# marja-w/gan-des-midi-music-gen

Measured on AMD Instinct MI355X. Metric: GAN training samples/sec (G+D step), higher is better.
Workload: dtype bf16; 1 GPU; SIMNN G/D iteration, synthetic 128x256 spectrogram windows; per_gpu_batch=256, global_batch=256, mode=faithful, parallelism=dp1

## Files before the change

### gan_des_midi_music_gen_amd/_lib.py

```python
import ctypes
import os
import threading

_PKG = os.path.dirname(os.path.abspath(__file__))
_TAG = os.environ.get("GDM_LIB_TAG", "")
LIB_PATH = os.path.join(_PKG, "libgdm_hip" + (f"_{_TAG}" if _TAG else "") + ".so")

F32, BF16 = 0, 1
ACT_NONE, ACT_RELU, ACT_LEAKY, ACT_SIGMOID = 0, 1, 2, 3
CRITERIA = {"bce": 0, "mse": 1, "l1": 2}
PCM_U8, PCM_S16, PCM_S24, PCM_S32, PCM_F32 = range(5)
PCM_BYTES = (1, 2, 3, 4, 4)

_c = ctypes
_P, _I, _L, _F, _Z = _c.c_void_p, _c.c_int, _c.c_int64, _c.c_float, _c.c_size_t

class LinearBnJob(_c.Structure):
    _fields_ = [(n, _P) for n in ("x", "w", "bias", "gamma", "beta", "running_mean", "running_var",
                                  "num_batches_tracked", "y_out", "out", "save_mean", "save_invstd")] + \
               [(n, _I) for n in ("M", "N", "K", "groups", "stat_repeats")]


class DcnnAdam(_c.Structure):
    _fields_ = [("param", _P * 6), ("exp_avg", _P * 6), ("exp_avg_sq", _P * 6), ("hyper", _P), ("done", _P)]


class ConcatJob(_c.Structure):
    _fields_ = [("a", _P), ("b", _P), ("out", _P), ("M", _I), ("Ka", _I), ("Kb", _I)]


SIGNATURES = {
    "gdm_last_error": (_c.c_char_p, []),
    "gdm_version": (_I, []),
    "gdm_arch": (_c.c_char_p, []),
    "gdm_build_flavor": (_I, []),
    "gdm_gemm": (_I, [_P, _I, _L, _L, _P, _I, _L, _L, _P, _I, _L, _L, _I, _I, _I, _P, _P, _I, _F, _I, _I, _P, _Z, _P]),
    "gdm_gemm_plan": (_I, [_P, _I, _L, _L, _P, _I, _L, _L, _P, _I, _L, _L, _I, _I, _I, _P, _I, _I, _P]),
    "gdm_bce_with_logits": (_I, [_P, _F, _I, _F, _P, _P, _I, _I, _P]),
    "gdm_criterion_loss": (_I, [_P, _F, _I, _I, _F, _P, _P, _I, _P]),
    "gdm_adam_step": (_I, [_P, _P, _P, _P, _L, _I, _F, _F, _F, _F, _F, _P]),
    "gdm_adam_step_dev": (_I, [_P, _P, _P, _P, _L, _P, _P]),
    "gdm_adam_step_dev_pc": (_I, [_P, _P, _P, _P, _I, _I, _I, _P, _I, _P, _I, _P]),
    "gdm_stft_frames": (_I, [_P, _I, _L, _L, _I, _I, _I, _P, _P]),
    "gdm_power_spectrum": (_I, [_P, _L, _I, _I, _P, _P]),
    "gdm_power_to_db": (_I, [_P, _I, _I, _I, _F, _F, _P, _P]),
    "gdm_pcm_to_float": (_I, [_P, _I, _I, _I, _L, _L, _L, _P, _P]),
    "gdm_pcm_stft_frames": (_I, [_P, _I, _I, _I, _L, _L, _L, _I, _L, _L, _I, _I, _I, _P, _P]),
    "gdm_bn_workspace_bytes": (_Z, [_I, _I]),
    "gdm_bn_act_fwd": (_I, [_P, _I, _I, _P, _P, _P, _P, _P, _F, _F, _I, _P, _I, _P, _P, _I, _P, _Z, _P]),
    "gdm_bn_act_bwd": (_I, [_P, _P, _I, _P, _I, _I, _P, _P, _P, _I, _P, _P, _P, _P, _Z, _P]),
    "gdm_bn_stats": (_I, [_P, _I, _I, _P, _P, _P, _F, _F, _P, _P, _P, _Z, _P]),
    "gdm_bn_partial_chunks": (_I, [_I]),
# ... 104 lines not shown
```

### gan_des_midi_music_gen_amd/csrc/gemm.hip

```cpp
#include "gemm_common.h"

namespace {

constexpr int BM = 64, BN = 64, NT = 256;

template <typename CT> struct GemmCfg;
template <> struct GemmCfg<float> { static constexpr int KT = 32, LD = 34; };
template <> struct GemmCfg<__bf16> { static constexpr int KT = 64, LD = 72; };

template <typename CT, typename TA, typename TB>
__global__ __launch_bounds__(NT) void gemm_kernel(GemmArgs g) {
  constexpr int KT = GemmCfg<CT>::KT, LD = GemmCfg<CT>::LD;
  __shared__ __attribute__((aligned(16))) CT smem[(BM + BN) * LD];
  CT* As = smem;
  CT* Bs = smem + BM * LD;
  const int t = threadIdx.x, l = t & 63, w = t >> 6, wm = w >> 1, wn = w & 1;
  const int lr = l & 15, lg = l >> 4;
  const int m0 = blockIdx.y * BM, n0 = blockIdx.x * BN;
  const int kbeg = blockIdx.z * g.k_per_split;
  const int kend = min(g.K, kbeg + g.k_per_split);
  const TA* __restrict__ A = (const TA*)g.A;
  const TB* __restrict__ B = (const TB*)g.B;
  const bool a_kfast = (g.sak == 1), b_kfast = (g.sbk == 1);
  f32x4 acc[2][2];
// ... 210 lines not shown
      gdm_set_error("gdm_gemm: split_k=%d needs %zu workspace bytes, got %zu", p.split_k, p.ws_bytes, workspace_bytes);
      return GDM_EWORKSPACE;
    }
  }
  GemmArgs g{A, sam, sak, B, sbk, sbn, C, c_dtype, scm, scn, M, N, K, bias_n, bias_m, act, slope,
             p.split_k, p.k_per_split, (float*)workspace};
  hipStream_t s = (hipStream_t)stream;
  if (p.kernel == GDM_GEMM_KERNEL_FAST_K32 || p.kernel == GDM_GEMM_KERNEL_FAST_K64) {
    rc = gdm_gemm_bf16_fast_launch(g, a_dtype, b_dtype, p, s);
    if (rc != GDM_OK) return rc;
    return launch_splitk_reduce(g, p, s);
  }
  return p.kernel == GDM_GEMM_KERNEL_BF16 ? launch_gemm<__bf16>(g, p, a_dtype, b_dtype, s)
                                          : launch_gemm<float>(g, p, a_dtype, b_dtype, s);
}
```

### gan_des_midi_music_gen_amd/csrc/gemm_bf16.hip

```cpp
#include "gemm_common.h"

namespace {

constexpr int BM = 128, BN = 128;

inline bool operand_ok(const void* p, int dtype, int64_t s_row, int64_t s_k, int rows, int K, bool* kmaj) {
  const int64_t esz = dtype == GDM_BF16 ? 2 : 4, epc = 16 / esz;
  if (((uintptr_t)p & 15) != 0) return false;
  if (s_k == 1 && s_row >= 1 && (s_row * esz) % 16 == 0 && K % epc == 0) {
    *kmaj = true;
    return ((int64_t)(rows - 1) * s_row + K) * esz < ((int64_t)1 << 31);
  }
  if (s_row == 1 && s_k >= 1 && (s_k * esz) % 16 == 0 && rows % epc == 0) {
    *kmaj = false;
    return ((int64_t)(K - 1) * s_k + rows) * esz < ((int64_t)1 << 31);
  }
  return false;
}

}

bool gdm_gemm_bf16_fast_ok(const GemmArgs& g, int a_dtype, int b_dtype, bool* a_kmaj, bool* b_kmaj) {
  if (!operand_ok(g.A, a_dtype, g.sam, g.sak, g.M, g.K, a_kmaj)) return false;
  if (!operand_ok(g.B, b_dtype, g.sbn, g.sbk, g.N, g.K, b_kmaj)) return false;
// ... 4 lines not shown
    if (g.bias_n && ((uintptr_t)g.bias_n & 15) != 0) return false;
  }
  if ((int64_t)g.M * g.N < 64 * 64) return false;
  return true;
}

bool gdm_gemm_bf16_fast_deep(int M, int N, int split_k, int k_per_split) {
  const int MT = (M + BM - 1) / BM, NTl = (N + BN - 1) / BN;
  const int outer = NTl * split_k;
  bool deep = split_k > 1 && (int64_t)outer * MT <= 512 && k_per_split >= 256;
  static const int force = GDM_TUNABLE("GDM_GEMM_VARIANT", -1);
  if (force >= 0) deep = force == 1;
  return deep;
}

int gdm_gemm_bf16_fast_launch(const GemmArgs& g, int a_dtype, int b_dtype, const GemmPlan& p, hipStream_t s) {
  const int MT = (g.M + BM - 1) / BM, NTl = (g.N + BN - 1) / BN;
  const int outer = NTl * g.split_k;
  dim3 grid((unsigned)(((outer + 7) / 8) * 8 * MT));
  const bool deep = p.kernel == GDM_GEMM_KERNEL_FAST_K64;
  auto* launch = a_dtype == GDM_BF16 ? (deep ? gdm_gemm_bf16_kt64_bf16a : gdm_gemm_bf16_kt32_bf16a)
                                     : (deep ? gdm_gemm_bf16_kt64_f32a : gdm_gemm_bf16_kt32_f32a);
  launch(g, p.a_kmaj, b_dtype, p.b_kmaj, grid, s);
  GDM_LAUNCH_OK("gdm_gemm(bf16 fast path)");
  return GDM_OK;
}
```

### gan_des_midi_music_gen_amd/csrc/gemm_bf16_kernel.h

```cpp
#pragma once
#include <type_traits>
#include "buffer_ops.h"
#include "gemm_common.h"

namespace {

constexpr int BM = 128, BN = 128, NT = 256;

__device__ __forceinline__ void wave_lds_sync() {
  __builtin_amdgcn_fence(__ATOMIC_RELEASE, "wavefront");
  __builtin_amdgcn_wave_barrier();
  __builtin_amdgcn_fence(__ATOMIC_ACQUIRE, "wavefront");
}

template <int ACT> __device__ __forceinline__ float act_const(float v, float slope) {
  if constexpr (ACT == GDM_ACT_RELU) return v > 0.f ? v : 0.f;
  else if constexpr (ACT == GDM_ACT_LEAKY) return v > 0.f ? v : v * slope;
  else if constexpr (ACT == GDM_ACT_SIGMOID) return 1.0f / (1.0f + expf(-v));
  else return v;
}

template <int KT> __device__ __forceinline__ int kswz(int row) { return KT == 64 ? ((row >> 1) & 7) : ((row >> 1) & 2); }
__device__ __forceinline__ int rswz(int k) { return (k & 3) | ((k >> 1) & 4); }

// ... 19 lines not shown
    if constexpr (KMAJ) {
      constexpr int CPR = KT / EPC;
      rl = c / CPR; kl = (c % CPR) * EPC;
      ln.off[i] = (uint32_t)(((int64_t)(r0 + rl) * ld + kl) * (int64_t)sizeof(T));
      ln.lds[i] = rl * KT + 8 * ((kl >> 3) ^ kswz<KT>(rl)) + (kl & 7);
    } else {
      constexpr int CPK = 128 / EPC;
      kl = c / CPK; rl = (c % CPK) * EPC;
      ln.off[i] = (uint32_t)(((int64_t)kl * ld + r0 + rl) * (int64_t)sizeof(T));
      ln.lds[i] = kl * 128 + (rl ^ (16 * rswz(kl)));
    }
    ln.kl[i] = (r0 + rl < rows) ? kl : -1;
  }
}

template <typename T, int KT, bool KMAJ>
__device__ __forceinline__ void stage_load(Stage<T, KT>& st, const Lane<T, KT>& ln, rsrc_t rs, int64_t ld, int k0,
                                           int kend) {
  const uint32_t kbytes = (uint32_t)((KMAJ ? (int64_t)k0 : (int64_t)k0 * ld) * (int64_t)sizeof(T));
#pragma unroll
  for (int i = 0; i < Stage<T, KT>::N; ++i) {
    const bool ok = ln.kl[i] >= 0 && k0 + ln.kl[i] < kend;
    st.v[i] = __builtin_bit_cast(f32x4, __builtin_amdgcn_raw_buffer_load_b128(rs, ok ? kbytes + ln.off[i] : BUF_OOB, 0, 0));
  }
}

template <typename T, int KT>
__device__ __forceinline__ void stage_store(const Stage<T, KT>& st, const Lane<T, KT>& ln, __bf16* __restrict__ img) {
#pragma unroll
  for (int i = 0; i < Stage<T, KT>::N; ++i) {
    if constexpr (sizeof(T) == 2) {
      *(f32x4*)(img + ln.lds[i]) = st.v[i];
    } else {
      bf16x4 h;
#pragma unroll
      for (int e = 0; e < 4; ++e) h[e] = (__bf16)st.v[i][e];
      *(bf16x4*)(img + ln.lds[i]) = h;
    }
// ... 3 lines not shown
template <int KT, bool KMAJ>
__device__ __forceinline__ bf16x8 frag_read(const __bf16* __restrict__ img, int row0, int kk, int lr, int lg) {
  if constexpr (KMAJ) {
    const int row = row0 + lr;
    return *(const bf16x8*)&img[row * KT + 8 * ((4 * kk + lg) ^ kswz<KT>(row))];
  } else {
    const int q = lr >> 2, p = lr & 3;
    const int kr = 32 * kk + 8 * lg + q;
    const int n = (row0 + 4 * p) ^ (16 * (q | (4 * (lg & 1))));
    const bf16x4 lo = lds_tr16(&img[kr * 128 + n]);
    const bf16x4 hi = lds_tr16(&img[(kr + 4) * 128 + n]);
    return __builtin_shufflevector(lo, hi, 0, 1, 2, 3, 4, 5, 6, 7);
  }
}

template <typename TA, bool A_KMAJ, typename TB, bool B_KMAJ, int KT, int DEPTH>
__global__ __launch_bounds__(NT) void gemm_bf16_fast(GemmArgs g) {
  constexpr int IMG = 128 * KT;
  __shared__ __attribute__((aligned(16))) __bf16 smem[2 * DEPTH * IMG];
  const int t = threadIdx.x, l = t & 63, w = t >> 6, wm = w >> 1, wn = w & 1;
  const int lr = l & 15, lg = l >> 4;
  const int MT = (g.M + BM - 1) / BM, NTl = (g.N + BN - 1) / BN;
  const int id = blockIdx.x;
  const int grp = id / (8 * MT), within = id % (8 * MT);
  const int outer = grp * 8 + (within & 7), mt = within >> 3;
  if (outer >= NTl * g.split_k) return;
  const int nt = outer % NTl, zs = outer / NTl;
  const int m0 = mt * BM, n0 = nt * BN;
  const int kstep = KT * g.split_k;
  const int kbeg = zs * KT;
  const int kend = g.K;
  const int64_t lda = A_KMAJ ? g.sam : g.sak;
  const int64_t ldb = B_KMAJ ? g.sbn : g.sbk;
  const rsrc_t ra = make_rsrc(g.A, (uint32_t)((A_KMAJ ? (int64_t)(g.M - 1) * lda + g.K : (int64_t)(g.K - 1) * lda + g.M) *
// ... 13 lines not shown

  auto multiply = [&](const __bf16* As, const __bf16* Bs) {
#pragma unroll
    for (int kk = 0; kk < KT / 32; ++kk) {
      bf16x8 a[4], b[4];
#pragma unroll
      for (int i = 0; i < 4; ++i) a[i] = frag_read<KT, A_KMAJ>(As, wm * 64 + 16 * i, kk, lr, lg);
#pragma unroll
      for (int j = 0; j < 4; ++j) b[j] = frag_read<KT, B_KMAJ>(Bs, wn * 64 + 16 * j, kk, lr, lg);
#pragma unroll
      for (int i = 0; i < 4; ++i)
#pragma unroll
        for (int j = 0; j < 4; ++j) acc[i][j] = mfma16(b[j], a[i], acc[i][j]);
    }
  };
  Stage<TA, KT> sa[DEPTH];
  Stage<TB, KT> sb[DEPTH];
  if constexpr (DEPTH == 2) {
    auto tile = [&](Stage<TA, KT>& xa, Stage<TB, KT>& xb, __bf16* As, int k0) {
      __bf16* Bs = As + IMG;
      stage_store<TA, KT>(xa, la, As);
      stage_store<TB, KT>(xb, lb, Bs);
      __syncthreads();
      stage_load<TA, KT, A_KMAJ>(xa, la, ra, lda, k0 + 2 * kstep, kend);
      stage_load<TB, KT, B_KMAJ>(xb, lb, rb, ldb, k0 + 2 * kstep, kend);
      multiply(As, Bs);
    };
    stage_load<TA, KT, A_KMAJ>(sa[0], la, ra, lda, kbeg, kend);
    stage_load<TB, KT, B_KMAJ>(sb[0], lb, rb, ldb, kbeg, kend);
    stage_load<TA, KT, A_KMAJ>(sa[1], la, ra, lda, kbeg + kstep, kend);
    stage_load<TB, KT, B_KMAJ>(sb[1], lb, rb, ldb, kbeg + kstep, kend);
    for (int k0 = kbeg; k0 < kend; k0 += 2 * kstep) {
      tile(sa[0], sb[0], smem, k0);
      tile(sa[DEPTH - 1], sb[DEPTH - 1], smem + 2 * IMG * (DEPTH - 1), k0 + kstep);
    }
  } else {
    __bf16* As = smem;
    __bf16* Bs = smem + IMG;
    stage_load<TA, KT, A_KMAJ>(sa[0], la, ra, lda, kbeg, kend);
    stage_load<TB, KT, B_KMAJ>(sb[0], lb, rb, ldb, kbeg, kend);
    for (int k0 = kbeg; k0 < kend; k0 += kstep) {
      __syncthreads();
      stage_store<TA, KT>(sa[0], la, As);
      stage_store<TB, KT>(sb[0], lb, Bs);
      __syncthreads();
      stage_load<TA, KT, A_KMAJ>(sa[0], la, ra, lda, k0 + kstep, kend);
      stage_load<TB, KT, B_KMAJ>(sb[0], lb, rb, ldb, k0 + kstep, kend);
      multiply(As, Bs);
    }
// ... 102 lines not shown
          if (g.bias_n) y += g.bias_n[n + r];
          if (g.bias_m) y += g.bias_m[m];
          store_from_f32(g.C, g.c_dtype, (int64_t)m * g.scm + n + r, act_const<ACT>(y, g.slope));
        }
      }
    }
  };
  switch (g.act) {
    case GDM_ACT_RELU: epilogue(std::integral_constant<int, GDM_ACT_RELU>{}); break;
    case GDM_ACT_LEAKY: epilogue(std::integral_constant<int, GDM_ACT_LEAKY>{}); break;
    case GDM_ACT_SIGMOID: epilogue(std::integral_constant<int, GDM_ACT_SIGMOID>{}); break;
    default: epilogue(std::integral_constant<int, GDM_ACT_NONE>{}); break;
  }
}

template <typename TA, int KT, int DEPTH, bool AK, typename TB>
void launch_b(const GemmArgs& g, bool b_kmaj, dim3 grid, hipStream_t s) {
  if (b_kmaj) hipLaunchKernelGGL((gemm_bf16_fast<TA, AK, TB, true, KT, DEPTH>), grid, dim3(NT), 0, s, g);
  else hipLaunchKernelGGL((gemm_bf16_fast<TA, AK, TB, false, KT, DEPTH>), grid, dim3(NT), 0, s, g);
}
template <typename TA, int KT, int DEPTH, bool AK>
void launch_a(const GemmArgs& g, int b_dtype, bool b_kmaj, dim3 grid, hipStream_t s) {
  if (b_dtype == GDM_BF16) launch_b<TA, KT, DEPTH, AK, __bf16>(g, b_kmaj, grid, s);
  else launch_b<TA, KT, DEPTH, AK, float>(g, b_kmaj, grid, s);
}
template <typename TA, int KT, int DEPTH>
void launch_instances(const GemmArgs& g, bool a_kmaj, int b_dtype, bool b_kmaj, dim3 grid, hipStream_t s) {
  if (a_kmaj) launch_a<TA, KT, DEPTH, true>(g, b_dtype, b_kmaj, grid, s);
  else launch_a<TA, KT, DEPTH, false>(g, b_dtype, b_kmaj, grid, s);
}

}
```

### gan_des_midi_music_gen_amd/csrc/gemm_bf16_kt32_bf16a.hip

```cpp
#include "gemm_bf16_kernel.h"

void gdm_gemm_bf16_kt32_bf16a(const GemmArgs& g, bool a_kmaj, int b_dtype, bool b_kmaj, dim3 grid, hipStream_t s) {
  launch_instances<__bf16, 32, 1>(g, a_kmaj, b_dtype, b_kmaj, grid, s);
}
```

### gan_des_midi_music_gen_amd/csrc/gemm_bf16_kt32_f32a.hip

```cpp
#include "gemm_bf16_kernel.h"

void gdm_gemm_bf16_kt32_f32a(const GemmArgs& g, bool a_kmaj, int b_dtype, bool b_kmaj, dim3 grid, hipStream_t s) {
  launch_instances<float, 32, 1>(g, a_kmaj, b_dtype, b_kmaj, grid, s);
}
```

### gan_des_midi_music_gen_amd/csrc/gemm_bf16_kt64_bf16a.hip

```cpp
#include "gemm_bf16_kernel.h"

void gdm_gemm_bf16_kt64_bf16a(const GemmArgs& g, bool a_kmaj, int b_dtype, bool b_kmaj, dim3 grid, hipStream_t s) {
  launch_instances<__bf16, 64, 2>(g, a_kmaj, b_dtype, b_kmaj, grid, s);
}
```

### gan_des_midi_music_gen_amd/csrc/gemm_bf16_kt64_f32a.hip

```cpp
#include "gemm_bf16_kernel.h"

void gdm_gemm_bf16_kt64_f32a(const GemmArgs& g, bool a_kmaj, int b_dtype, bool b_kmaj, dim3 grid, hipStream_t s) {
  launch_instances<float, 64, 2>(g, a_kmaj, b_dtype, b_kmaj, grid, s);
}
```

### gan_des_midi_music_gen_amd/csrc/gemm_common.h

```cpp
#pragma once
#include "gdm_common.h"

struct GemmArgs {
  const void* A; int64_t sam, sak;
  const void* B; int64_t sbk, sbn;
  void* C; int c_dtype; int64_t scm, scn;
  int M, N, K;
  const float* bias_n; const float* bias_m; int act; float slope;
  int split_k, k_per_split; float* ws;
};

__device__ __forceinline__ void gemm_epilogue_store(const GemmArgs& g, int m, int n, float v) {
  if (g.bias_n) v += g.bias_n[n];
  if (g.bias_m) v += g.bias_m[m];
  v = apply_act(v, g.act, g.slope);
  store_from_f32(g.C, g.c_dtype, (int64_t)m * g.scm + (int64_t)n * g.scn, v);
}

struct GemmPlan {
  int kernel;
  bool a_kmaj, b_kmaj;
  int split_k, k_per_split;
  int reduce;
  size_t ws_bytes;
};

bool gdm_gemm_bf16_fast_ok(const GemmArgs& g, int a_dtype, int b_dtype, bool* a_kmaj, bool* b_kmaj);
bool gdm_gemm_bf16_fast_deep(int M, int N, int split_k, int k_per_split);
int gdm_gemm_bf16_fast_launch(const GemmArgs& g, int a_dtype, int b_dtype, const GemmPlan& p, hipStream_t s);
void gdm_gemm_bf16_kt32_bf16a(const GemmArgs& g, bool a_kmaj, int b_dtype, bool b_kmaj, dim3 grid, hipStream_t s);
void gdm_gemm_bf16_kt32_f32a(const GemmArgs& g, bool a_kmaj, int b_dtype, bool b_kmaj, dim3 grid, hipStream_t s);
void gdm_gemm_bf16_kt64_bf16a(const GemmArgs& g, bool a_kmaj, int b_dtype, bool b_kmaj, dim3 grid, hipStream_t s);
void gdm_gemm_bf16_kt64_f32a(const GemmArgs& g, bool a_kmaj, int b_dtype, bool b_kmaj, dim3 grid, hipStream_t s);
constexpr int GDM_GEMM_FAST_KT = 64;
```

### gan_des_midi_music_gen_amd/functional.py

```python
import contextlib

import torch

from . import ops
from .ops import ACT_LEAKY, ACT_NONE, ACT_RELU, ACT_SIGMOID, BF16, F32

_DEFAULT = {"dtype": F32}
_NAMES = {"fp32": F32, "f32": F32, "float32": F32, "bf16": BF16, "bfloat16": BF16, F32: F32, BF16: BF16}


def set_compute_dtype(name):
    _DEFAULT["dtype"] = _NAMES[name]


def get_compute_dtype():
    return _DEFAULT["dtype"]


@contextlib.contextmanager
def compute_dtype(name):
    old = _DEFAULT["dtype"]
    _DEFAULT["dtype"] = _NAMES[name]
    try:
        yield
# ... 17 lines not shown
    return pack, wf1p


def simnn_disc_features(x, w1, b1, pack, b2, wf1p, bf1, dt, trunk_out=None):
    if trunk_out is None:
        x = _f32c(x)
        p1, code1 = ops.simnn_conv1_fwd(x, w1, b1, dt)
    else:
        p1, code1 = trunk_out
    p2, code2 = ops.simnn_conv2_fwd(p1, pack, b2)
    b = p1.shape[0]
    flat = p2.view(b, -1)
    if flat.shape[1] != wf1p.shape[1]:
        raise ValueError(f"Discriminator.fc1 expects {wf1p.shape[1]} features but this input gives {flat.shape[1]} "
                         "(construct Discriminator(input_hw=...) for this geometry)")
    h1 = ops.gemm(flat, wf1p.t(), bias_n=bf1, act=ACT_RELU, compute=dt)
    return h1, (x, p1, code1, flat, code2, h1)


def simnn_disc_forward(x, w1, b1, pack, b2, wf1p, bf1, wf2, bf2, dt, trunk_out=None):
    h1, saved = simnn_disc_features(x, w1, b1, pack, b2, wf1p, bf1, dt, trunk_out)
    p = ops.gemm(h1, wf2.t(), bias_n=bf2, act=ACT_SIGMOID, compute=dt)
    return p, saved + (p,)


def simnn_disc_backward_from_dh1(saved, dh1, pack, wf1p, dt, out=None, x_pair=None, w1_for_dx=None):
    x, p1, code1, flat, code2 = saved[:5]
    b = p1.shape[0]
    o = out if out is not None else [None] * 8
    n, k = wf1p.shape
    dwf1p = ops.gemm(dh1.t(), flat, compute=dt)
    dwf1 = ops.permute_pc(dwf1p, n, k // 32, 32, out=o[4]).view(n, k)
    dflat = ops.gemm(dh1, wf1p, compute=dt, out_dtype=dt)
    h1s, w1s = p1.shape[1], p1.shape[2]
    dp2 = dflat.view(b, h1s // 2, w1s // 2, 32)
    dw2, db2 = ops.simnn_conv2_bwd_weight(dp2, code2, p1, out=None if out is None else (o[2], o[3]))
    x0, x1 = x_pair if x_pair is not None else (x, None)
    dw1, db1, dp1 = ops.simnn_conv2_bwd_fused(dp2, code2, pack, code1, x0, x1,
                                              out=None if out is None else (o[0], o[1]), want_dp1=w1_for_dx is not None)
    dx = None
    if w1_for_dx is not None:
        dx = ops.simnn_conv1_bwd_data(dp1, code1, w1_for_dx.contiguous(), x0.shape[1], x0.shape[2])
    return dw1, db1, dw2, db2, dwf1, dx


def simnn_disc_backward(saved, dz, pack, wf1p, wf2, dt, out=None, x_pair=None, w1_for_dx=None):
    h1 = saved[5]
    b = h1.shape[0]
# ... 486 lines not shown
```

### gan_des_midi_music_gen_amd/ops.py

```python
import contextlib
import ctypes
import threading

import torch

from . import _lib
from ._lib import ACT_LEAKY, ACT_NONE, ACT_RELU, ACT_SIGMOID, BF16, CRITERIA, F32, GdmError, check
from ._lib import PCM_BYTES, PCM_F32, PCM_S16, PCM_S24, PCM_S32, PCM_U8

_TORCH_DT = {F32: torch.float32, BF16: torch.bfloat16}


def torch_dtype(dt):
    return _TORCH_DT[dt]


def gdm_dtype(t):
    if t.dtype == torch.float32:
        return F32
    if t.dtype == torch.bfloat16:
        return BF16
    raise GdmError(f"unsupported tensor dtype {t.dtype} (fp32 or bf16 only)")


# ... 69 lines not shown
        _ws_pinned.add(key)
    return buf


def default_split_k(m, n, k, compute):
    tile, kt = (128, 32) if compute == BF16 else (64, 32)
    tiles = ((m + tile - 1) // tile) * ((n + tile - 1) // tile)
    ktiles = (k + kt - 1) // kt
    if tiles >= 128 or ktiles < 32:
        return 1
    target = 256 if compute == BF16 else 768
    return max(1, min(ktiles // 8, (target + tiles - 1) // tiles))


def gemm(a, b, *, bias_n=None, bias_m=None, act=ACT_NONE, slope=0.0, out_dtype=None, compute=F32, split_k=None,
         out=None):
    _need_gpu(a, b, bias_n, bias_m, out)
    assert a.dim() == 2 and b.dim() == 2 and a.shape[1] == b.shape[0], (a.shape, b.shape)
    m, k = a.shape
    n = b.shape[1]
    if out is None:
        out = torch.empty((m, n), dtype=_TORCH_DT[F32 if out_dtype is None else out_dtype], device=a.device)
    assert out.shape == (m, n)
    if split_k is None:
        split_k = default_split_k(m, n, k, compute)
    ws, ws_bytes = None, 0
    if split_k > 1:
        ws_bytes = split_k * m * n * 4
        ws = workspace(ws_bytes, a.device)
    lib = _lib.load()
    _call("gdm_gemm", _p(a), gdm_dtype(a), a.stride(0), a.stride(1), _p(b), gdm_dtype(b), b.stride(0), b.stride(1),
                       _p(out), gdm_dtype(out), out.stride(0), out.stride(1), m, n, k, _p(bias_n), _p(bias_m), act,
                       float(slope), compute, split_k, _p(ws), ws_bytes, _stream())
    return out


GEMM_KERNELS = ("generic_f32", "generic_bf16", "fast_k32", "fast_k64")
GEMM_REDUCES = ("none", "vector", "scalar")


def gemm_plan_raw(a_ptr, a_dtype, sam, sak, b_ptr, b_dtype, sbk, sbn, c_ptr, c_dtype, scm, scn, m, n, k, bias_n_ptr,
                  compute, split_k):
    out = (ctypes.c_int64 * 7)()
    lib = _lib.load()
    check(lib.gdm_gemm_plan(a_ptr, a_dtype, sam, sak, b_ptr, b_dtype, sbk, sbn, c_ptr, c_dtype, scm, scn, m, n, k,
                            bias_n_ptr or None, compute, split_k, ctypes.cast(out, ctypes.c_void_p)), "gdm_gemm_plan")
    return dict(kernel=GEMM_KERNELS[out[0]], a_kmajor=bool(out[1]), b_kmajor=bool(out[2]), split_k=int(out[3]),
                k_per_split=int(out[4]), reduce=GEMM_REDUCES[out[5]], workspace_bytes=int(out[6]))


def gemm_plan(a, b, *, bias_n=None, bias_m=None, act=ACT_NONE, slope=0.0, out_dtype=None, compute=F32, split_k=None,
              out=None):
    assert a.dim() == 2 and b.dim() == 2 and a.shape[1] == b.shape[0], (a.shape, b.shape)
    m, k = a.shape
    n = b.shape[1]
    if split_k is None:
        split_k = default_split_k(m, n, k, compute)
    if out is None:
        c_ptr, c_dtype, scm, scn = 1 << 12, (F32 if out_dtype is None else out_dtype), n, 1
    else:
        assert out.shape == (m, n)
        c_ptr, c_dtype, scm, scn = out.data_ptr(), gdm_dtype(out), out.stride(0), out.stride(1)
    return gemm_plan_raw(a.data_ptr(), gdm_dtype(a), a.stride(0), a.stride(1), b.data_ptr(), gdm_dtype(b), b.stride(0),
                         b.stride(1), c_ptr, c_dtype, scm, scn, m, n, k,
                         bias_n.data_ptr() if bias_n is not None else None, compute, split_k)


def bce_with_logits(x, target, *, grad_scale=1.0, want_grad=True, fuse_sigmoid_backward=False, loss_out=None,
                    accumulate_loss=False, dx_out=None):
    _need_gpu(x, loss_out, dx_out)
    x = x.reshape(-1)
    assert x.dtype == torch.float32 and x.is_contiguous()
    loss = loss_out if loss_out is not None else torch.empty(1, dtype=torch.float32, device=x.device)
    dx = dx_out if dx_out is not None else (torch.empty_like(x) if want_grad else None)
    if dx is not None:
        assert dx.is_contiguous() and dx.numel() == x.numel() and dx.dtype == torch.float32
    _call("gdm_bce_with_logits", _p(x), float(target), x.numel(), float(grad_scale), _p(loss), _p(dx),
                                           1 if fuse_sigmoid_backward else 0, 1 if accumulate_loss else 0, _stream())
    return loss, dx

# ... 975 lines not shown
```

### gan_des_midi_music_gen_amd/train.py

```python
import torch

from . import dp
from . import functional as Fn
from . import ops


class FlatBuffers:

    ALIGN = 64

    def __init__(self, params, extra=0, local=0):
        params = [p for p in params]
        assert params, "no parameters"
        dev = params[0].device
        self.params = params
        self.numel = sum(p.numel() for p in params)
        big = max(range(len(params)), key=lambda i: params[i].numel())
        order = [i for i in range(len(params)) if i != big] + [big]
        n_small = self.numel - params[big].numel()
        assert extra % 4 == 0 and 0 <= local <= extra
        self.n_small = (n_small + self.ALIGN - 1) // self.ALIGN * self.ALIGN
        self.n_pad = self.n_small - n_small
        self.n_extra = extra
        self.n_local = local
# ... 292 lines not shown
    def _features_head(self, x, trunk, n0, y0, y1, loss_out, grad_out=None, want_grad=True):
        w1, b1, _w2, b2, _wf1, bf1, wf2, bf2 = self.d.views
        pack, wf1p = self._operands()
        hid, saved = Fn.simnn_disc_features(x, w1, b1, pack, b2, wf1p, bf1, self.dt, trunk_out=trunk)
        prob, dh, _ = ops.simnn_head(hid, wf2, bf2, n0, y0, y1, loss_out=loss_out, want_grad=want_grad,
                                     grad_out=grad_out, dh_dtype=self.dt)
        return saved, dh, (hid, prob)

    def _disc_features_head(self, trunk):
        gv = self.d.grad_views
        return self._features_head(None, trunk, trunk[0].shape[0] // 2, 0.9, 0.1, self.loss_d,
                                   grad_out=(gv[6], gv[7], gv[5]))

    def _fc1_dw(self, saved, dh, outs):
        n, k = self._prepared[1].shape
        ops.gemm(dh.t(), saved[3], compute=self.dt, out=outs[4].view(n, k))

    def _backward_rest(self, saved, dh, outs, x_pair, keep):
        _x, p1, code1, _flat, code2 = saved[:5]
        pack, wf1p = self._prepared
        dflat = ops.gemm(dh, wf1p, compute=self.dt, out_dtype=self.dt)
        dp2 = dflat.view(p1.shape[0], p1.shape[1] // 2, p1.shape[2] // 2, 32)
        keep.append(dflat)
        ops.simnn_conv2_bwd_weight(dp2, code2, p1, out=(outs[2], outs[3]))
        ops.simnn_conv2_bwd_fused(dp2, code2, pack, code1, x_pair[0], x_pair[1], out=(outs[0], outs[1]))

    def _d_backward(self, saved, dh, outs, x_pair, keep, fork=True):
        main = torch.cuda.current_stream()
        side = self._streams(saved[1].device, fork)
        if side:
            side[1].wait_stream(main)
        with torch.cuda.stream(side[1] if side else main):
            self._fc1_dw(saved, dh, outs)
            if self.world > 1 and outs is self.d.grad_views:
                self._reduce_big_async()
        self._backward_rest(saved, dh, outs, x_pair, keep)
# ... 483 lines not shown
```

### include/gdm.h

```cpp
#ifndef GDM_H
#define GDM_H
#include <stddef.h>
#include <stdint.h>

#ifdef __cplusplus
extern "C" {
#endif

enum { GDM_F32 = 0, GDM_BF16 = 1 };
enum { GDM_ACT_NONE = 0, GDM_ACT_RELU = 1, GDM_ACT_LEAKY = 2, GDM_ACT_SIGMOID = 3 };
enum { GDM_OK = 0, GDM_EINVAL = -1, GDM_ELAUNCH = -2, GDM_EWORKSPACE = -3 };
enum { GDM_CRIT_BCE_LOGITS = 0, GDM_CRIT_MSE = 1, GDM_CRIT_L1 = 2 };

const char* gdm_last_error(void);
int gdm_version(void);
const char* gdm_arch(void);
int gdm_build_flavor(void);

int gdm_gemm(const void* A, int a_dtype, int64_t sam, int64_t sak,
             const void* B, int b_dtype, int64_t sbk, int64_t sbn,
             void* C, int c_dtype, int64_t scm, int64_t scn,
             int M, int N, int K,
             const float* bias_n, const float* bias_m, int act, float slope,
             int compute_dtype, int split_k, void* workspace, size_t workspace_bytes, void* stream);

enum { GDM_GEMM_KERNEL_F32 = 0, GDM_GEMM_KERNEL_BF16 = 1, GDM_GEMM_KERNEL_FAST_K32 = 2, GDM_GEMM_KERNEL_FAST_K64 = 3 };
enum { GDM_GEMM_REDUCE_NONE = 0, GDM_GEMM_REDUCE_VECTOR = 1, GDM_GEMM_REDUCE_SCALAR = 2 };
enum { GDM_GEMM_PLAN_KERNEL = 0, GDM_GEMM_PLAN_A_KMAJOR = 1, GDM_GEMM_PLAN_B_KMAJOR = 2, GDM_GEMM_PLAN_SPLIT_K = 3,
       GDM_GEMM_PLAN_K_PER_SPLIT = 4, GDM_GEMM_PLAN_REDUCE = 5, GDM_GEMM_PLAN_WORKSPACE_BYTES = 6,
       GDM_GEMM_PLAN_FIELDS = 7 };
int gdm_gemm_plan(const void* A, int a_dtype, int64_t sam, int64_t sak,
                  const void* B, int b_dtype, int64_t sbk, int64_t sbn,
                  const void* C, int c_dtype, int64_t scm, int64_t scn,
                  int M, int N, int K, const float* bias_n, int compute_dtype, int split_k, int64_t* plan);

int gdm_bce_with_logits(const float* x, float target, int n, float grad_scale, float* loss, float* dx,
                        int fuse_sigmoid_backward, int accumulate_loss, void* stream);

int gdm_criterion_loss(const float* x, float target, int n, int criterion, float grad_scale, float* loss, float* dx,
                       int accumulate_loss, void* stream);

int gdm_adam_step(float* p, const float* g, float* m, float* v, int64_t n, int step, float lr, float beta1,
                  float beta2, float eps, float grad_scale, void* stream);

int gdm_adam_step_dev(float* p, const float* g, float* m, float* v, int64_t n, float* hyper, void* stream);
int gdm_adam_step_dev_pc(float* p, const float* g_pc, float* m, float* v, int N, int C, int P, void* shadow_pc,
                         int shadow_dtype, float* hyper, int advance_step, void* stream);

size_t gdm_bn_workspace_bytes(int rows, int channels);
// ... 250 lines not shown
```

Measured before the change: 418,200 samples/s.

## Add deeper register-prefetch streaming GEMM variants for discriminator fc1 GEMMs

Adds new bf16 GEMM kernel instances that keep three register stages of global loads in flight ahead of the LDS stores (AHEAD=3) while using one or two LDS buffers, with the k offset passed as the buffer-load soffset. A selector maps eligible fast-path plans to these variants, and the discriminator fc1 forward, weight-grad and data-grad GEMMs now request them. The aim is to hide global memory latency on these large-K, bandwidth-bound GEMMs. The cost is higher register pressure, which may reduce occupancy.

```diff
diff --git a/gan_des_midi_music_gen_amd/_lib.py b/gan_des_midi_music_gen_amd/_lib.py
--- a/gan_des_midi_music_gen_amd/_lib.py
+++ b/gan_des_midi_music_gen_amd/_lib.py
@@ -36,6 +36,9 @@
     "gdm_build_flavor": (_I, []),
     "gdm_gemm": (_I, [_P, _I, _L, _L, _P, _I, _L, _L, _P, _I, _L, _L, _I, _I, _I, _P, _P, _I, _F, _I, _I, _P, _Z, _P]),
     "gdm_gemm_plan": (_I, [_P, _I, _L, _L, _P, _I, _L, _L, _P, _I, _L, _L, _I, _I, _I, _P, _I, _I, _P]),
+    "gdm_gemm_stream": (_I, [_P, _I, _L, _L, _P, _I, _L, _L, _P, _I, _L, _L, _I, _I, _I, _P, _P, _I, _F, _I, _I, _P, _Z,
+                             _P]),
+    "gdm_gemm_stream_plan": (_I, [_P, _I, _L, _L, _P, _I, _L, _L, _P, _I, _L, _L, _I, _I, _I, _P, _I, _I, _P]),
     "gdm_bce_with_logits": (_I, [_P, _F, _I, _F, _P, _P, _I, _I, _P]),
     "gdm_criterion_loss": (_I, [_P, _F, _I, _I, _F, _P, _P, _I, _P]),
     "gdm_adam_step": (_I, [_P, _P, _P, _P, _L, _I, _F, _F, _F, _F, _F, _P]),
diff --git a/gan_des_midi_music_gen_amd/csrc/gemm.hip b/gan_des_midi_music_gen_amd/csrc/gemm.hip
--- a/gan_des_midi_music_gen_amd/csrc/gemm.hip
+++ b/gan_des_midi_music_gen_amd/csrc/gemm.hip
@@ -248,3 +248,40 @@
   return p.kernel == GDM_GEMM_KERNEL_BF16 ? launch_gemm<__bf16>(g, p, a_dtype, b_dtype, s)
                                           : launch_gemm<float>(g, p, a_dtype, b_dtype, s);
 }
+
+extern "C" int gdm_gemm_stream_plan(const void* A, int a_dtype, int64_t sam, int64_t sak, const void* B, int b_dtype,
+                                    int64_t sbk, int64_t sbn, const void* C, int c_dtype, int64_t scm, int64_t scn, int M,
+                                    int N, int K, const float* bias_n, int compute_dtype, int split_k, int64_t* plan) {
+  int rc = gdm_gemm_plan(A, a_dtype, sam, sak, B, b_dtype, sbk, sbn, C, c_dtype, scm, scn, M, N, K, bias_n, compute_dtype,
+                         split_k, plan);
+  if (rc != GDM_OK) return rc;
+  plan[GDM_GEMM_PLAN_KERNEL] = gdm_gemm_bf16_stream_kernel((int)plan[GDM_GEMM_PLAN_KERNEL], a_dtype,
+                                                           plan[GDM_GEMM_PLAN_A_KMAJOR] != 0, b_dtype,
+                                                           plan[GDM_GEMM_PLAN_B_KMAJOR] != 0);
+  return GDM_OK;
+}
+
+extern "C" int gdm_gemm_stream(const void* A, int a_dtype, int64_t sam, int64_t sak, const void* B, int b_dtype,
+                               int64_t sbk, int64_t sbn, void* C, int c_dtype, int64_t scm, int64_t scn, int M, int N,
+                               int K, const float* bias_n, const float* bias_m, int act, float slope, int compute_dtype,
+                               int split_k, void* workspace, size_t workspace_bytes, void* stream) {
+  GemmPlan p;
+  int rc = gemm_plan(A, a_dtype, sam, sak, B, b_dtype, sbk, sbn, C, c_dtype, scm, scn, M, N, K, bias_n, compute_dtype,
+                     split_k, &p);
+  if (rc != GDM_OK) return rc;
+  p.kernel = gdm_gemm_bf16_stream_kernel(p.kernel, a_dtype, p.a_kmaj, b_dtype, p.b_kmaj);
+  if (p.kernel != GDM_GEMM_KERNEL_STREAM_K32 && p.kernel != GDM_GEMM_KERNEL_STREAM_K64)
+    return gdm_gemm(A, a_dtype, sam, sak, B, b_dtype, sbk, sbn, C, c_dtype, scm, scn, M, N, K, bias_n, bias_m, act, slope,
+                    compute_dtype, split_k, workspace, workspace_bytes, stream);
+  GDM_REQUIRE(act >= GDM_ACT_NONE && act <= GDM_ACT_SIGMOID, "gdm_gemm: bad activation %d", act);
+  if (p.split_k > 1 && (workspace == nullptr || workspace_bytes < p.ws_bytes)) {
+    gdm_set_error("gdm_gemm: split_k=%d needs %zu workspace bytes, got %zu", p.split_k, p.ws_bytes, workspace_bytes);
+    return GDM_EWORKSPACE;
+  }
+  GemmArgs g{A, sam, sak, B, sbk, sbn, C, c_dtype, scm, scn, M, N, K, bias_n, bias_m, act, slope,
+             p.split_k, p.k_per_split, (float*)workspace};
+  hipStream_t s = (hipStream_t)stream;
+  rc = gdm_gemm_bf16_fast_launch(g, a_dtype, b_dtype, p, s);
+  if (rc != GDM_OK) return rc;
+  return launch_splitk_reduce(g, p, s);
+}
diff --git a/gan_des_midi_music_gen_amd/csrc/gemm_bf16.hip b/gan_des_midi_music_gen_amd/csrc/gemm_bf16.hip
--- a/gan_des_midi_music_gen_amd/csrc/gemm_bf16.hip
+++ b/gan_des_midi_music_gen_amd/csrc/gemm_bf16.hip
@@ -42,14 +42,28 @@
   return deep;
 }
 
+int gdm_gemm_bf16_stream_kernel(int kernel, int a_dtype, bool a_kmaj, int b_dtype, bool b_kmaj) {
+  if (b_dtype != GDM_BF16) return kernel;
+  if (kernel == GDM_GEMM_KERNEL_FAST_K32 && !a_kmaj && !b_kmaj) return GDM_GEMM_KERNEL_STREAM_K32;
+  if (kernel == GDM_GEMM_KERNEL_FAST_K64 && a_dtype == GDM_BF16 && a_kmaj && b_kmaj) return GDM_GEMM_KERNEL_STREAM_K64;
+  return kernel;
+}
+
 int gdm_gemm_bf16_fast_launch(const GemmArgs& g, int a_dtype, int b_dtype, const GemmPlan& p, hipStream_t s) {
   const int MT = (g.M + BM - 1) / BM, NTl = (g.N + BN - 1) / BN;
   const int outer = NTl * g.split_k;
   dim3 grid((unsigned)(((outer + 7) / 8) * 8 * MT));
-  const bool deep = p.kernel == GDM_GEMM_KERNEL_FAST_K64;
-  auto* launch = a_dtype == GDM_BF16 ? (deep ? gdm_gemm_bf16_kt64_bf16a : gdm_gemm_bf16_kt32_bf16a)
-                                     : (deep ? gdm_gemm_bf16_kt64_f32a : gdm_gemm_bf16_kt32_f32a);
-  launch(g, p.a_kmaj, b_dtype, p.b_kmaj, grid, s);
+  if (p.kernel == GDM_GEMM_KERNEL_STREAM_K32) {
+    if (a_dtype == GDM_BF16) gdm_gemm_bf16_stream_kt32_bf16a(g, grid, s);
+    else gdm_gemm_bf16_stream_kt32_f32a(g, grid, s);
+  } else if (p.kernel == GDM_GEMM_KERNEL_STREAM_K64) {
+    gdm_gemm_bf16_stream_kt64_bf16a(g, grid, s);
+  } else {
+    const bool deep = p.kernel == GDM_GEMM_KERNEL_FAST_K64;
+    auto* launch = a_dtype == GDM_BF16 ? (deep ? gdm_gemm_bf16_kt64_bf16a : gdm_gemm_bf16_kt32_bf16a)
+                                       : (deep ? gdm_gemm_bf16_kt64_f32a : gdm_gemm_bf16_kt32_f32a);
+    launch(g, p.a_kmaj, b_dtype, p.b_kmaj, grid, s);
+  }
   GDM_LAUNCH_OK("gdm_gemm(bf16 fast path)");
   return GDM_OK;
 }
diff --git a/gan_des_midi_music_gen_amd/csrc/gemm_bf16_kernel.h b/gan_des_midi_music_gen_amd/csrc/gemm_bf16_kernel.h
--- a/gan_des_midi_music_gen_amd/csrc/gemm_bf16_kernel.h
+++ b/gan_des_midi_music_gen_amd/csrc/gemm_bf16_kernel.h
@@ -57,14 +57,17 @@
   }
 }
 
-template <typename T, int KT, bool KMAJ>
+template <typename T, int KT, bool KMAJ, bool KS = false>
 __device__ __forceinline__ void stage_load(Stage<T, KT>& st, const Lane<T, KT>& ln, rsrc_t rs, int64_t ld, int k0,
                                            int kend) {
   const uint32_t kbytes = (uint32_t)((KMAJ ? (int64_t)k0 : (int64_t)k0 * ld) * (int64_t)sizeof(T));
 #pragma unroll
   for (int i = 0; i < Stage<T, KT>::N; ++i) {
     const bool ok = ln.kl[i] >= 0 && k0 + ln.kl[i] < kend;
-    st.v[i] = __builtin_bit_cast(f32x4, __builtin_amdgcn_raw_buffer_load_b128(rs, ok ? kbytes + ln.off[i] : BUF_OOB, 0, 0));
+    if constexpr (KS)
+      st.v[i] = __builtin_bit_cast(f32x4, __builtin_amdgcn_raw_buffer_load_b128(rs, ok ? ln.off[i] : BUF_OOB, kbytes, 0));
+    else
+      st.v[i] = __builtin_bit_cast(f32x4, __builtin_amdgcn_raw_buffer_load_b128(rs, ok ? kbytes + ln.off[i] : BUF_OOB, 0, 0));
   }
 }
 
@@ -98,10 +101,11 @@
   }
 }
 
-template <typename TA, bool A_KMAJ, typename TB, bool B_KMAJ, int KT, int DEPTH>
+template <typename TA, bool A_KMAJ, typename TB, bool B_KMAJ, int KT, int LDSB, int AHEAD>
 __global__ __launch_bounds__(NT) void gemm_bf16_fast(GemmArgs g) {
+  static_assert((LDSB == 1 || LDSB == 2) && AHEAD >= LDSB, "one or two LDS buffers, at least as many register stages");
   constexpr int IMG = 128 * KT;
-  __shared__ __attribute__((aligned(16))) __bf16 smem[2 * DEPTH * IMG];
+  __shared__ __attribute__((aligned(16))) __bf16 smem[2 * LDSB * IMG];
   const int t = threadIdx.x, l = t & 63, w = t >> 6, wm = w >> 1, wn = w & 1;
   const int lr = l & 15, lg = l >> 4;
   const int MT = (g.M + BM - 1) / BM, NTl = (g.N + BN - 1) / BN;
@@ -145,9 +149,36 @@
         for (int j = 0; j < 4; ++j) acc[i][j] = mfma16(b[j], a[i], acc[i][j]);
     }
   };
-  Stage<TA, KT> sa[DEPTH];
-  Stage<TB, KT> sb[DEPTH];
-  if constexpr (DEPTH == 2) {
+  Stage<TA, KT> sa[AHEAD];
+  Stage<TB, KT> sb[AHEAD];
+  if constexpr (AHEAD > LDSB) {
+    constexpr int U = AHEAD % LDSB == 0 ? AHEAD : AHEAD * LDSB;
+    auto tile = [&](Stage<TA, KT>& xa, Stage<TB, KT>& xb, __bf16* As, int k0) {
+      __bf16* Bs = As + IMG;
+      if constexpr (LDSB == 1) __syncthreads();
+      stage_store<TA, KT>(xa, la, As);
+      stage_store<TB, KT>(xb, lb, Bs);
+      __syncthreads();
+      stage_load<TA, KT, A_KMAJ, true>(xa, la, ra, lda, k0 + AHEAD * kstep, kend);
+      stage_load<TB, KT, B_KMAJ, true>(xb, lb, rb, ldb, k0 + AHEAD * kstep, kend);
+      multiply(As, Bs);
+    };
+#pragma unroll
+    for (int i = 0; i < AHEAD; ++i) {
+      stage_load<TA, KT, A_KMAJ, true>(sa[i], la, ra, lda, kbeg + i * kstep, kend);
+      stage_load<TB, KT, B_KMAJ, true>(sb[i], lb, rb, ldb, kbeg + i * kstep, kend);
+    }
+    int k0 = kbeg;
+    for (; k0 + (U - 1) * kstep < kend; k0 += U * kstep) {
+#pragma unroll
+      for (int u = 0; u < U; ++u) tile(sa[u % AHEAD], sb[u % AHEAD], smem + 2 * IMG * (u % LDSB), k0 + u * kstep);
+    }
+#pragma unroll
+    for (int u = 0; u < U - 1; ++u) {
+      if (k0 + u * kstep >= kend) break;
+      tile(sa[u % AHEAD], sb[u % AHEAD], smem + 2 * IMG * (u % LDSB), k0 + u * kstep);
+    }
+  } else if constexpr (LDSB == 2) {
     auto tile = [&](Stage<TA, KT>& xa, Stage<TB, KT>& xb, __bf16* As, int k0) {
       __bf16* Bs = As + IMG;
       stage_store<TA, KT>(xa, la, As);
@@ -163,7 +194,7 @@
     stage_load<TB, KT, B_KMAJ>(sb[1], lb, rb, ldb, kbeg + kstep, kend);
     for (int k0 = kbeg; k0 < kend; k0 += 2 * kstep) {
       tile(sa[0], sb[0], smem, k0);
-      tile(sa[DEPTH - 1], sb[DEPTH - 1], smem + 2 * IMG * (DEPTH - 1), k0 + kstep);
+      tile(sa[1], sb[1], smem + 2 * IMG, k0 + kstep);
     }
   } else {
     __bf16* As = smem;
@@ -296,20 +327,24 @@
   }
 }
 
-template <typename TA, int KT, int DEPTH, bool AK, typename TB>
+template <typename TA, bool AK, typename TB, bool BK, int KT, int LDSB, int AHEAD>
+void launch_one(const GemmArgs& g, dim3 grid, hipStream_t s) {
+  hipLaunchKernelGGL((gemm_bf16_fast<TA, AK, TB, BK, KT, LDSB, AHEAD>), grid, dim3(NT), 0, s, g);
+}
+template <typename TA, int KT, int LDSB, int AHEAD, bool AK, typename TB>
 void launch_b(const GemmArgs& g, bool b_kmaj, dim3 grid, hipStream_t s) {
-  if (b_kmaj) hipLaunchKernelGGL((gemm_bf16_fast<TA, AK, TB, true, KT, DEPTH>), grid, dim3(NT), 0, s, g);
-  else hipLaunchKernelGGL((gemm_bf16_fast<TA, AK, TB, false, KT, DEPTH>), grid, dim3(NT), 0, s, g);
-}
-template <typename TA, int KT, int DEPTH, bool AK>
+  if (b_kmaj) hipLaunchKernelGGL((gemm_bf16_fast<TA, AK, TB, true, KT, LDSB, AHEAD>), grid, dim3(NT), 0, s, g);
+  else hipLaunchKernelGGL((gemm_bf16_fast<TA, AK, TB, false, KT, LDSB, AHEAD>), grid, dim3(NT), 0, s, g);
+}
+template <typename TA, int KT, int LDSB, int AHEAD, bool AK>
 void launch_a(const GemmArgs& g, int b_dtype, bool b_kmaj, dim3 grid, hipStream_t s) {
-  if (b_dtype == GDM_BF16) launch_b<TA, KT, DEPTH, AK, __bf16>(g, b_kmaj, grid, s);
-  else launch_b<TA, KT, DEPTH, AK, float>(g, b_kmaj, grid, s);
-}
-template <typename TA, int KT, int DEPTH>
+  if (b_dtype == GDM_BF16) launch_b<TA, KT, LDSB, AHEAD, AK, __bf16>(g, b_kmaj, grid, s);
+  else launch_b<TA, KT, LDSB, AHEAD, AK, float>(g, b_kmaj, grid, s);
+}
+template <typename TA, int KT, int LDSB, int AHEAD>
 void launch_instances(const GemmArgs& g, bool a_kmaj, int b_dtype, bool b_kmaj, dim3 grid, hipStream_t s) {
-  if (a_kmaj) launch_a<TA, KT, DEPTH, true>(g, b_dtype, b_kmaj, grid, s);
-  else launch_a<TA, KT, DEPTH, false>(g, b_dtype, b_kmaj, grid, s);
-}
-
-}
+  if (a_kmaj) launch_a<TA, KT, LDSB, AHEAD, true>(g, b_dtype, b_kmaj, grid, s);
+  else launch_a<TA, KT, LDSB, AHEAD, false>(g, b_dtype, b_kmaj, grid, s);
+}
+
+}
diff --git a/gan_des_midi_music_gen_amd/csrc/gemm_bf16_kt32_bf16a.hip b/gan_des_midi_music_gen_amd/csrc/gemm_bf16_kt32_bf16a.hip
--- a/gan_des_midi_music_gen_amd/csrc/gemm_bf16_kt32_bf16a.hip
+++ b/gan_des_midi_music_gen_amd/csrc/gemm_bf16_kt32_bf16a.hip
@@ -1,5 +1,5 @@
 #include "gemm_bf16_kernel.h"
 
 void gdm_gemm_bf16_kt32_bf16a(const GemmArgs& g, bool a_kmaj, int b_dtype, bool b_kmaj, dim3 grid, hipStream_t s) {
-  launch_instances<__bf16, 32, 1>(g, a_kmaj, b_dtype, b_kmaj, grid, s);
+  launch_instances<__bf16, 32, 1, 1>(g, a_kmaj, b_dtype, b_kmaj, grid, s);
 }
diff --git a/gan_des_midi_music_gen_amd/csrc/gemm_bf16_kt32_f32a.hip b/gan_des_midi_music_gen_amd/csrc/gemm_bf16_kt32_f32a.hip
--- a/gan_des_midi_music_gen_amd/csrc/gemm_bf16_kt32_f32a.hip
+++ b/gan_des_midi_music_gen_amd/csrc/gemm_bf16_kt32_f32a.hip
@@ -1,5 +1,5 @@
 #include "gemm_bf16_kernel.h"
 
 void gdm_gemm_bf16_kt32_f32a(const GemmArgs& g, bool a_kmaj, int b_dtype, bool b_kmaj, dim3 grid, hipStream_t s) {
-  launch_instances<float, 32, 1>(g, a_kmaj, b_dtype, b_kmaj, grid, s);
+  launch_instances<float, 32, 1, 1>(g, a_kmaj, b_dtype, b_kmaj, grid, s);
 }
diff --git a/gan_des_midi_music_gen_amd/csrc/gemm_bf16_kt64_bf16a.hip b/gan_des_midi_music_gen_amd/csrc/gemm_bf16_kt64_bf16a.hip
--- a/gan_des_midi_music_gen_amd/csrc/gemm_bf16_kt64_bf16a.hip
+++ b/gan_des_midi_music_gen_amd/csrc/gemm_bf16_kt64_bf16a.hip
@@ -1,5 +1,5 @@
 #include "gemm_bf16_kernel.h"
 
 void gdm_gemm_bf16_kt64_bf16a(const GemmArgs& g, bool a_kmaj, int b_dtype, bool b_kmaj, dim3 grid, hipStream_t s) {
-  launch_instances<__bf16, 64, 2>(g, a_kmaj, b_dtype, b_kmaj, grid, s);
+  launch_instances<__bf16, 64, 2, 2>(g, a_kmaj, b_dtype, b_kmaj, grid, s);
 }
diff --git a/gan_des_midi_music_gen_amd/csrc/gemm_bf16_kt64_f32a.hip b/gan_des_midi_music_gen_amd/csrc/gemm_bf16_kt64_f32a.hip
--- a/gan_des_midi_music_gen_amd/csrc/gemm_bf16_kt64_f32a.hip
+++ b/gan_des_midi_music_gen_amd/csrc/gemm_bf16_kt64_f32a.hip
@@ -1,5 +1,5 @@
 #include "gemm_bf16_kernel.h"
 
 void gdm_gemm_bf16_kt64_f32a(const GemmArgs& g, bool a_kmaj, int b_dtype, bool b_kmaj, dim3 grid, hipStream_t s) {
-  launch_instances<float, 64, 2>(g, a_kmaj, b_dtype, b_kmaj, grid, s);
+  launch_instances<float, 64, 2, 2>(g, a_kmaj, b_dtype, b_kmaj, grid, s);
 }
diff --git a/gan_des_midi_music_gen_amd/csrc/gemm_bf16_stream_kt32_bf16a.hip b/gan_des_midi_music_gen_amd/csrc/gemm_bf16_stream_kt32_bf16a.hip
--- /dev/null
+++ b/gan_des_midi_music_gen_amd/csrc/gemm_bf16_stream_kt32_bf16a.hip
@@ -0,0 +1,5 @@
+#include "gemm_bf16_kernel.h"
+
+void gdm_gemm_bf16_stream_kt32_bf16a(const GemmArgs& g, dim3 grid, hipStream_t s) {
+  launch_one<__bf16, false, __bf16, false, 32, 1, 3>(g, grid, s);
+}
diff --git a/gan_des_midi_music_gen_amd/csrc/gemm_bf16_stream_kt32_f32a.hip b/gan_des_midi_music_gen_amd/csrc/gemm_bf16_stream_kt32_f32a.hip
--- /dev/null
+++ b/gan_des_midi_music_gen_amd/csrc/gemm_bf16_stream_kt32_f32a.hip
@@ -0,0 +1,5 @@
+#include "gemm_bf16_kernel.h"
+
+void gdm_gemm_bf16_stream_kt32_f32a(const GemmArgs& g, dim3 grid, hipStream_t s) {
+  launch_one<float, false, __bf16, false, 32, 1, 3>(g, grid, s);
+}
diff --git a/gan_des_midi_music_gen_amd/csrc/gemm_bf16_stream_kt64_bf16a.hip b/gan_des_midi_music_gen_amd/csrc/gemm_bf16_stream_kt64_bf16a.hip
--- /dev/null
+++ b/gan_des_midi_music_gen_amd/csrc/gemm_bf16_stream_kt64_bf16a.hip
@@ -0,0 +1,5 @@
+#include "gemm_bf16_kernel.h"
+
+void gdm_gemm_bf16_stream_kt64_bf16a(const GemmArgs& g, dim3 grid, hipStream_t s) {
+  launch_one<__bf16, true, __bf16, true, 64, 2, 3>(g, grid, s);
+}
diff --git a/gan_des_midi_music_gen_amd/csrc/gemm_common.h b/gan_des_midi_music_gen_amd/csrc/gemm_common.h
--- a/gan_des_midi_music_gen_amd/csrc/gemm_common.h
+++ b/gan_des_midi_music_gen_amd/csrc/gemm_common.h
@@ -32,4 +32,8 @@
 void gdm_gemm_bf16_kt32_f32a(const GemmArgs& g, bool a_kmaj, int b_dtype, bool b_kmaj, dim3 grid, hipStream_t s);
 void gdm_gemm_bf16_kt64_bf16a(const GemmArgs& g, bool a_kmaj, int b_dtype, bool b_kmaj, dim3 grid, hipStream_t s);
 void gdm_gemm_bf16_kt64_f32a(const GemmArgs& g, bool a_kmaj, int b_dtype, bool b_kmaj, dim3 grid, hipStream_t s);
+int gdm_gemm_bf16_stream_kernel(int kernel, int a_dtype, bool a_kmaj, int b_dtype, bool b_kmaj);
+void gdm_gemm_bf16_stream_kt32_bf16a(const GemmArgs& g, dim3 grid, hipStream_t s);
+void gdm_gemm_bf16_stream_kt32_f32a(const GemmArgs& g, dim3 grid, hipStream_t s);
+void gdm_gemm_bf16_stream_kt64_bf16a(const GemmArgs& g, dim3 grid, hipStream_t s);
 constexpr int GDM_GEMM_FAST_KT = 64;
diff --git a/gan_des_midi_music_gen_amd/functional.py b/gan_des_midi_music_gen_amd/functional.py
--- a/gan_des_midi_music_gen_amd/functional.py
+++ b/gan_des_midi_music_gen_amd/functional.py
@@ -55,7 +55,7 @@
     if flat.shape[1] != wf1p.shape[1]:
         raise ValueError(f"Discriminator.fc1 expects {wf1p.shape[1]} features but this input gives {flat.shape[1]} "
                          "(construct Discriminator(input_hw=...) for this geometry)")
-    h1 = ops.gemm(flat, wf1p.t(), bias_n=bf1, act=ACT_RELU, compute=dt)
+    h1 = ops.gemm(flat, wf1p.t(), bias_n=bf1, act=ACT_RELU, compute=dt, stream=True)
     return h1, (x, p1, code1, flat, code2, h1)
 
 
@@ -70,9 +70,9 @@
     b = p1.shape[0]
     o = out if out is not None else [None] * 8
     n, k = wf1p.shape
-    dwf1p = ops.gemm(dh1.t(), flat, compute=dt)
+    dwf1p = ops.gemm(dh1.t(), flat, compute=dt, stream=True)
     dwf1 = ops.permute_pc(dwf1p, n, k // 32, 32, out=o[4]).view(n, k)
-    dflat = ops.gemm(dh1, wf1p, compute=dt, out_dtype=dt)
+    dflat = ops.gemm(dh1, wf1p, compute=dt, out_dtype=dt, stream=True)
     h1s, w1s = p1.shape[1], p1.shape[2]
     dp2 = dflat.view(b, h1s // 2, w1s // 2, 32)
     dw2, db2 = ops.simnn_conv2_bwd_weight(dp2, code2, p1, out=None if out is None else (o[2], o[3]))
diff --git a/gan_des_midi_music_gen_amd/ops.py b/gan_des_midi_music_gen_amd/ops.py
--- a/gan_des_midi_music_gen_amd/ops.py
+++ b/gan_des_midi_music_gen_amd/ops.py
@@ -107,7 +107,7 @@
 
 
 def gemm(a, b, *, bias_n=None, bias_m=None, act=ACT_NONE, slope=0.0, out_dtype=None, compute=F32, split_k=None,
-         out=None):
+         out=None, stream=False):
     _need_gpu(a, b, bias_n, bias_m, out)
     assert a.dim() == 2 and b.dim() == 2 and a.shape[1] == b.shape[0], (a.shape, b.shape)
     m, k = a.shape
@@ -122,28 +122,29 @@
         ws_bytes = split_k * m * n * 4
         ws = workspace(ws_bytes, a.device)
     lib = _lib.load()
-    _call("gdm_gemm", _p(a), gdm_dtype(a), a.stride(0), a.stride(1), _p(b), gdm_dtype(b), b.stride(0), b.stride(1),
-                       _p(out), gdm_dtype(out), out.stride(0), out.stride(1), m, n, k, _p(bias_n), _p(bias_m), act,
-                       float(slope), compute, split_k, _p(ws), ws_bytes, _stream())
+    _call("gdm_gemm_stream" if stream else "gdm_gemm", _p(a), gdm_dtype(a), a.stride(0), a.stride(1), _p(b), gdm_dtype(b),
+          b.stride(0), b.stride(1), _p(out), gdm_dtype(out), out.stride(0), out.stride(1), m, n, k, _p(bias_n),
+          _p(bias_m), act, float(slope), compute, split_k, _p(ws), ws_bytes, _stream())
     return out
 
 
-GEMM_KERNELS = ("generic_f32", "generic_bf16", "fast_k32", "fast_k64")
+GEMM_KERNELS = ("generic_f32", "generic_bf16", "fast_k32", "fast_k64", "stream_k32", "stream_k64")
 GEMM_REDUCES = ("none", "vector", "scalar")
 
 
 def gemm_plan_raw(a_ptr, a_dtype, sam, sak, b_ptr, b_dtype, sbk, sbn, c_ptr, c_dtype, scm, scn, m, n, k, bias_n_ptr,
-                  compute, split_k):
+                  compute, split_k, stream=False):
     out = (ctypes.c_int64 * 7)()
     lib = _lib.load()
-    check(lib.gdm_gemm_plan(a_ptr, a_dtype, sam, sak, b_ptr, b_dtype, sbk, sbn, c_ptr, c_dtype, scm, scn, m, n, k,
-                            bias_n_ptr or None, compute, split_k, ctypes.cast(out, ctypes.c_void_p)), "gdm_gemm_plan")
+    fn = lib.gdm_gemm_stream_plan if stream else lib.gdm_gemm_plan
+    check(fn(a_ptr, a_dtype, sam, sak, b_ptr, b_dtype, sbk, sbn, c_ptr, c_dtype, scm, scn, m, n, k,
+             bias_n_ptr or None, compute, split_k, ctypes.cast(out, ctypes.c_void_p)), "gdm_gemm_plan")
     return dict(kernel=GEMM_KERNELS[out[0]], a_kmajor=bool(out[1]), b_kmajor=bool(out[2]), split_k=int(out[3]),
                 k_per_split=int(out[4]), reduce=GEMM_REDUCES[out[5]], workspace_bytes=int(out[6]))
 
 
 def gemm_plan(a, b, *, bias_n=None, bias_m=None, act=ACT_NONE, slope=0.0, out_dtype=None, compute=F32, split_k=None,
-              out=None):
+              out=None, stream=False):
     assert a.dim() == 2 and b.dim() == 2 and a.shape[1] == b.shape[0], (a.shape, b.shape)
     m, k = a.shape
     n = b.shape[1]
@@ -156,7 +157,11 @@
         c_ptr, c_dtype, scm, scn = out.data_ptr(), gdm_dtype(out), out.stride(0), out.stride(1)
     return gemm_plan_raw(a.data_ptr(), gdm_dtype(a), a.stride(0), a.stride(1), b.data_ptr(), gdm_dtype(b), b.stride(0),
                          b.stride(1), c_ptr, c_dtype, scm, scn, m, n, k,
-                         bias_n.data_ptr() if bias_n is not None else None, compute, split_k)
+                         bias_n.data_ptr() if bias_n is not None else None, compute, split_k, stream)
+
+
+def gemm_stream_plan(a, b, **kw):
+    return gemm_plan(a, b, stream=True, **kw)
 
 
 def bce_with_logits(x, target, *, grad_scale=1.0, want_grad=True, fuse_sigmoid_backward=False, loss_out=None,
diff --git a/gan_des_midi_music_gen_amd/train.py b/gan_des_midi_music_gen_amd/train.py
--- a/gan_des_midi_music_gen_amd/train.py
+++ b/gan_des_midi_music_gen_amd/train.py
@@ -330,12 +330,12 @@
 
     def _fc1_dw(self, saved, dh, outs):
         n, k = self._prepared[1].shape
-        ops.gemm(dh.t(), saved[3], compute=self.dt, out=outs[4].view(n, k))
+        ops.gemm(dh.t(), saved[3], compute=self.dt, out=outs[4].view(n, k), stream=True)
 
     def _backward_rest(self, saved, dh, outs, x_pair, keep):
         _x, p1, code1, _flat, code2 = saved[:5]
         pack, wf1p = self._prepared
-        dflat = ops.gemm(dh, wf1p, compute=self.dt, out_dtype=self.dt)
+        dflat = ops.gemm(dh, wf1p, compute=self.dt, out_dtype=self.dt, stream=True)
         dp2 = dflat.view(p1.shape[0], p1.shape[1] // 2, p1.shape[2] // 2, 32)
         keep.append(dflat)
         ops.simnn_conv2_bwd_weight(dp2, code2, p1, out=(outs[2], outs[3]))
diff --git a/include/gdm.h b/include/gdm.h
--- a/include/gdm.h
+++ b/include/gdm.h
@@ -24,7 +24,8 @@
              const float* bias_n, const float* bias_m, int act, float slope,
              int compute_dtype, int split_k, void* workspace, size_t workspace_bytes, void* stream);
 
-enum { GDM_GEMM_KERNEL_F32 = 0, GDM_GEMM_KERNEL_BF16 = 1, GDM_GEMM_KERNEL_FAST_K32 = 2, GDM_GEMM_KERNEL_FAST_K64 = 3 };
+enum { GDM_GEMM_KERNEL_F32 = 0, GDM_GEMM_KERNEL_BF16 = 1, GDM_GEMM_KERNEL_FAST_K32 = 2, GDM_GEMM_KERNEL_FAST_K64 = 3,
+       GDM_GEMM_KERNEL_STREAM_K32 = 4, GDM_GEMM_KERNEL_STREAM_K64 = 5  };
 enum { GDM_GEMM_REDUCE_NONE = 0, GDM_GEMM_REDUCE_VECTOR = 1, GDM_GEMM_REDUCE_SCALAR = 2 };
 enum { GDM_GEMM_PLAN_KERNEL = 0, GDM_GEMM_PLAN_A_KMAJOR = 1, GDM_GEMM_PLAN_B_KMAJOR = 2, GDM_GEMM_PLAN_SPLIT_K = 3,
        GDM_GEMM_PLAN_K_PER_SPLIT = 4, GDM_GEMM_PLAN_REDUCE = 5, GDM_GEMM_PLAN_WORKSPACE_BYTES = 6,
@@ -33,6 +34,17 @@
                   const void* B, int b_dtype, int64_t sbk, int64_t sbn,
                   const void* C, int c_dtype, int64_t scm, int64_t scn,
                   int M, int N, int K, const float* bias_n, int compute_dtype, int split_k, int64_t* plan);
+
+int gdm_gemm_stream(const void* A, int a_dtype, int64_t sam, int64_t sak,
+                    const void* B, int b_dtype, int64_t sbk, int64_t sbn,
+                    void* C, int c_dtype, int64_t scm, int64_t scn,
+                    int M, int N, int K,
+                    const float* bias_n, const float* bias_m, int act, float slope,
+                    int compute_dtype, int split_k, void* workspace, size_t workspace_bytes, void* stream);
+int gdm_gemm_stream_plan(const void* A, int a_dtype, int64_t sam, int64_t sak,
+                         const void* B, int b_dtype, int64_t sbk, int64_t sbn,
+                         const void* C, int c_dtype, int64_t scm, int64_t scn,
+                         int M, int N, int K, const float* bias_n, int compute_dtype, int split_k, int64_t* plan);
 
 int gdm_bce_with_logits(const float* x, float target, int n, float grad_scale, float* loss, float* dx,
                         int fuse_sigmoid_backward, int accumulate_loss, void* stream);
```

New measurement: 420,400 samples/s (median of 6 runs). About the same (+0.5%).
